# zgspose/PAVENet

Measured on AMD Instinct MI355X. Metric: clips/sec (T=7, 800x1344) fwd, higher is better.
Workload: dtype f32 (exact 3-term bf16 split on the bf16 MFMA)

## Files before the change

pavenet_amd/csrc/pave_gemm_dma.hip:

```cpp
#include <hip/hip_runtime.h>
#include <type_traits>
#include <stdint.h>

#include "pave_hip.h"
#include "pave_internal.h"
#include "pave_enc_math.h"

namespace {

typedef __bf16 bf16x8 __attribute__((ext_vector_type(8)));
typedef float f32x16 __attribute__((ext_vector_type(16)));
typedef unsigned u32x4 __attribute__((ext_vector_type(4)));
typedef float f32x4 __attribute__((ext_vector_type(4)));

constexpr int QBM = 128;
constexpr int QNS = 3;
constexpr int QCST = 36;

struct QConv {
  int H, W, Cin, Ho, Wo, stride;
  unsigned rcp;
};
struct QOut {
  float* out2;
// ... 125 lines not shown
}
#define PAVE_CLOCK_BEGIN(kind) diag_stagger(); const ClockStamp pave_cs(kind)
#define PAVE_CLOCK_END() pave_cs.end()
#define PAVE_PROBE_DROP_STORES() (g_diag_stagger == -1 || g_diag_stagger == -3 || g_diag_stagger == -5)
#define PAVE_PROBE_CACHED_A() (g_diag_stagger == -2 || g_diag_stagger == -3)
#define PAVE_PROBE_NO_CHAIN_SYNC() (g_diag_stagger == -4 || g_diag_stagger == -5)
#define PAVE_PROBE_NT_STORES() (g_diag_stagger == -6)
#define PAVE_PROBE_FREE_SPLIT() (g_diag_stagger == -7)
#else
#define PAVE_CLOCK_BEGIN(kind)
#define PAVE_CLOCK_END()
#define PAVE_PROBE_DROP_STORES() false
#define PAVE_PROBE_CACHED_A() false
#define PAVE_PROBE_NO_CHAIN_SYNC() false
#define PAVE_PROBE_NT_STORES() false
#define PAVE_PROBE_FREE_SPLIT() false
#endif

template <int TN, int WN, int KIND, bool ABIAS, bool LNORM, bool WIDE = false, int EPI = 0, int RM = 1, int PL = 3,
          bool HT = false, int IO = 0>
__device__ __forceinline__ void gemm_q_body(
    const float* __restrict__ A, const uint16_t* __restrict__ Wp, const float* __restrict__ bias,
    const float* residual, float* out, const int M, const int K, const int N, const int relu,
    const float* __restrict__ a_bias, const QConv g, const QOut os, const QLn ln,
    const float* __restrict__ A2 = nullptr, const int tile_m0 = -1, const int tile_n0 = 0,
    const QEpi* epi = nullptr) {
  constexpr int NWAVE = 4 * WN;
  constexpr int BN = WN * TN * 32;
  constexpr int BM = QBM * RM;
  constexpr bool AH = (IO & 1) != 0, OH = (IO & 2) != 0;
  static_assert(!AH || (PL == 1 && KIND == 0 && !ABIAS && RM == 1), "fp16 A rows: fp16 operand mode, plain rows");
  static_assert(!OH || (PL == 1 && !LNORM && EPI == 0 && !HT && RM == 1), "fp16 output: plain epilogue");
  constexpr int A_STAGE = AH ? BM * 32 : BM * 64;
  static_assert(RM == 1 || (RM == 2 && WN == 1 && !WIDE && !LNORM && EPI == 0), "two row tiles per wave: narrow form");
  static_assert(PL == 3 || PL == 1, "operand planes: 3 (bf16 split) or 1 (fp16)");
  constexpr int W_STAGE = PL * BN * 32;
  constexpr int STAGE = A_STAGE + W_STAGE;
  constexpr int NA = A_STAGE / 1024;
  constexpr int NWI = W_STAGE / 1024;
  constexpr int NDI = NA + NWI;
  constexpr int QMAX = (NDI + NWAVE - 1) / NWAVE;
  constexpr int QMIN = NDI / NWAVE;
  constexpr int QA = (NA + NWAVE - 1) / NWAVE;
  constexpr int NS = WIDE ? 2 : QNS;
  constexpr int EPI_OFF = 0;
  constexpr int STAT_OFF = NS * STAGE;
  constexpr int TQ = WIDE ? 2 : (HT ? 1 : TN);
  static_assert(!HT || (TN == 2 && WN == 1 && RM == 1 && !WIDE && !LNORM && EPI == 0 && PL == 3),
                "half-tail form: 64-column planes, one row tile per wave, 3 planes");
  static_assert(!WIDE || (TN == 8 && WN == 1 && !ABIAS), "wide form: 32 x 256 per wave");
  constexpr int ABOFF = STAT_OFF + (LNORM ? 2 * QBM * WN * 4 : 0);
  static_assert(NA % NWAVE == 0, "A DMA instructions divide evenly over the waves");
  static_assert(!LNORM || KIND == 0, "LayerNorm epilogue: plain row GEMM only");
  static_assert(KIND >= 0 && KIND <= 4, "row source");
  extern __shared__ __attribute__((aligned(1024))) unsigned char smem[];

  const int tid = threadIdx.x, lane = tid & 63;
  const int wave = __builtin_amdgcn_readfirstlane(tid >> 6);
  const int wm = wave / WN, wn = wave % WN;
  const int lr = lane & 31, kh = lane >> 5;
  const int ntiles = N / BN;
  const int ttot = ((M + BM - 1) / BM) * ntiles;
  const int per = ttot >> 3, rem = ttot & 7;
  const unsigned lds0 = (unsigned)(size_t)(__attribute__((address_space(3))) unsigned char*)smem;
  const int s0 = os.ks_slabs > 0 ? (int)blockIdx.y * os.ks_slabs : 0;
  const int nslabs = os.ks_slabs > 0 ? min(os.ks_slabs, K / 16 - s0) : K / 16;
  const long long w_slab = (long long)PL * N * 32;
  const unsigned char* const w_base = reinterpret_cast<const unsigned char*>(Wp);

  int m0 = 0, n0 = 0;
  unsigned a_voff[QA];
  unsigned a2_voff[QA];
  const unsigned char* a2_base = reinterpret_cast<const unsigned char*>(A2);
  int a_iy0[QA], a_ix0[QA];
  const float* a_img[QA];
  unsigned a_mask[QA];
  i32x4 a_rsrc;
  if (KIND == 1) {
    const unsigned long long ab = reinterpret_cast<unsigned long long>(A);
    a_rsrc.x = __builtin_amdgcn_readfirstlane((int)(unsigned)ab);
// ... 82 lines not shown
        dma16_buf(ok ? a_voff[q] + toff : 0xffffff00u, a_rsrc, dst);
      } else if (KIND == 2) {
        const int k0 = slab * 16;
        const int tap = k0 / g.Cin, c0 = k0 - tap * g.Cin;
        const int ky = tap / 3, kx = tap - ky * 3;
        const int iy = a_iy0[q] + ky, ix = a_ix0[q] + kx;
        const bool ok = tap < 9 && iy >= 0 && iy < g.H && ix >= 0 && ix < g.W;
        const float* src = ok ? a_img[q] + ((long long)iy * g.W + ix) * g.Cin + c0
                              : reinterpret_cast<const float*>(g_zero_chunk);
        dma16_flat(src, dst);
      } else if (KIND == 4) {
        const int s1 = g.Cin >> 4;
        if (slab < s1) dma16(a_voff[q], a_base + (long long)slab * 64, dst);
        else dma16(a2_voff[q], a2_base + (long long)(slab - s1) * 64, dst);
      } else {
        dma16(a_voff[q], a_base + (long long)slab * (AH ? 32 : 64), dst);
      }
    }
#pragma unroll
    for (int q = QA; q < QMAX; ++q) {
      const int j = wave + NWAVE * (q - QA);
      if (NWI % NWAVE == 0 || j < NWI)
        dma16(w_voff[q - QA], w_base + slab * w_slab, sl + A_STAGE + j * 1024);
    }
  };

  const int sw = (lr >> 2) & 3;
  const int a_rd0 = AH ? (wm * 32 + lr) * 32 + ((kh ^ ((lr >> 3) & 1)) * 16)
                       : (wm * 32 * RM + lr) * 64 + (((2 * kh) ^ sw) * 16);
  const int a_rd1 = a_rd0 ^ 16;
  const int w_rd = A_STAGE + (wn * TN * 32 + lr) * 32 + ((kh ^ ((lr >> 3) & 1)) * 16);

  f32x16 acc[RM * TN];
  f32x4 raw[RM][2];
  u32x4 apl[2][RM][PL];
  u32x4 wf[2][PL][TQ];
  const float* const ab_lds = reinterpret_cast<const float*>(smem + ABOFF);

  auto read_raw = [&](const int stage) {
    const unsigned char* st = smem + stage * STAGE;
#pragma unroll
    for (int rt = 0; rt < RM; ++rt) {
      raw[rt][0] = *reinterpret_cast<const f32x4*>(st + a_rd0 + rt * 2048);
      if constexpr (!AH) raw[rt][1] = *reinterpret_cast<const f32x4*>(st + a_rd1 + rt * 2048);
    }
  };
  auto read_wq = [&](const int stage, const int quarter, const int set) {
    const unsigned char* st = smem + stage * STAGE;
#pragma unroll
    for (int p = 0; p < PL; ++p)
#pragma unroll
      for (int j = 0; j < TQ; ++j)
        wf[set][p][j] =
            *reinterpret_cast<const u32x4*>(st + w_rd + (p * BN + (quarter * TQ + j) * 32) * 32);
  };
  u32x4 wtA[PL], wtB[PL], wt[PL];
  f32x4 acct[2];
  const int w_rdt = A_STAGE + (32 + (lane & 15)) * 32 + (((((lane >> 4) & 1)) ^ ((lane >> 3) & 1)) * 16);
  auto read_tail = [&](const int stage, u32x4 (&dst)[PL]) {
    const unsigned char* st = smem + stage * STAGE;
#pragma unroll
    for (int p = 0; p < PL; ++p) dst[p] = *reinterpret_cast<const u32x4*>(st + w_rdt + p * BN * 32);
  };
  auto read_frags = [&](const int stage, const int set) {
    read_raw(stage);
    read_wq(stage, 0, set);
    if constexpr (HT) {
      if (set == 0) read_tail(stage, wtA);
      else read_tail(stage, wtB);
    }
  };
  auto merge_tail = [&]() {
    if constexpr (HT) {
#pragma unroll
      for (int p = 0; p < PL; ++p)
#pragma unroll
        for (int i = 0; i < 4; ++i) wt[p][i] = lane < 32 ? wtA[p][i] : wtB[p][i];
    }
  };
  auto tail_pair = [&]() {
    if constexpr (HT) {
      typedef unsigned u32x2 __attribute__((ext_vector_type(2)));
#pragma unroll
      for (int p = 0; p < PL; ++p)
#pragma unroll
        for (int i = 0; i < 4; ++i) {
          u32x2 r = __builtin_amdgcn_permlane32_swap(apl[0][0][p][i], apl[1][0][p][i], false, false);
          r = __builtin_amdgcn_permlane16_swap(r.x, r.y, false, false);
          apl[0][0][p][i] = r.x, apl[1][0][p][i] = r.y;
        }
#pragma unroll
      for (int o = 2; o >= 0; --o)
#pragma unroll
        for (int pa = 0; pa <= o; ++pa)
#pragma unroll
          for (int hh = 0; hh < 2; ++hh)
            acct[hh] = __builtin_amdgcn_mfma_f32_16x16x32_bf16(
                __builtin_bit_cast(bf16x8, apl[hh][0][pa]), __builtin_bit_cast(bf16x8, wt[o - pa]), acct[hh], 0, 0, 0);
    }
  };
  auto split_raw = [&](const int slab, const int set) {
#pragma unroll
   for (int rt = 0; rt < RM; ++rt) {
    f32x4 lo = raw[rt][0], hi = raw[rt][1];
    if (ABIAS) {
      const f32x4 b0 = *reinterpret_cast<const f32x4*>(ab_lds + slab * 16 + kh * 8);
      const f32x4 b1 = *reinterpret_cast<const f32x4*>(ab_lds + slab * 16 + kh * 8 + 4);
#pragma unroll
      for (int i = 0; i < 4; ++i) {
        lo[i] = fmaxf(lo[i] + b0[i], 0.f);
        hi[i] = fmaxf(hi[i] + b1[i], 0.f);
      }
    }
    if constexpr (AH) {
      apl[set][rt][0] = __builtin_bit_cast(u32x4, lo);
    } else if constexpr (PL == 3) {
      if (PAVE_PROBE_FREE_SPLIT()) {
        apl[set][rt][0] = __builtin_bit_cast(u32x4, lo);
        apl[set][rt][1] = __builtin_bit_cast(u32x4, hi);
        apl[set][rt][2] = __builtin_bit_cast(u32x4, lo);
      } else
      split8(lo, hi, apl[set][rt]);
    } else {
      apl[set][rt][0] = u32x4{pack_rne_f16(lo.x, lo.y), pack_rne_f16(lo.z, lo.w), pack_rne_f16(hi.x, hi.y),
                              pack_rne_f16(hi.z, hi.w)};
    }
   }
  };
  auto mma = [&](const int set, const int o) {
    if constexpr (PL == 1) {
      if (o != 0) return;
#pragma unroll
      for (int rt = 0; rt < RM; ++rt)
#pragma unroll
        for (int j = 0; j < TQ; ++j)
          acc[rt * TN + j] = __builtin_amdgcn_mfma_f32_32x32x16_f16(
              __builtin_bit_cast(f16x8, apl[set][rt][0]), __builtin_bit_cast(f16x8, wf[set][0][j]),
              acc[rt * TN + j], 0, 0, 0);
    } else {
#pragma unroll
    for (int pa = 0; pa <= o; ++pa)
#pragma unroll
      for (int rt = 0; rt < RM; ++rt)
#pragma unroll
        for (int j = 0; j < TQ; ++j) {
          acc[rt * TN + j] = __builtin_amdgcn_mfma_f32_32x32x16_bf16(
              __builtin_bit_cast(bf16x8, apl[set][rt][pa]), __builtin_bit_cast(bf16x8, wf[set][o - pa][j]),
              acc[rt * TN + j], 0, 0, 0);
        }
    }
  };
  auto mma_q = [&](const int aset, const int wset, const int quarter) {
    if constexpr (PL == 1) {
#pragma unroll
      for (int j = 0; j < TQ; ++j)
        acc[quarter * TQ + j] = __builtin_amdgcn_mfma_f32_32x32x16_f16(
            __builtin_bit_cast(f16x8, apl[aset][0][0]), __builtin_bit_cast(f16x8, wf[wset][0][j]),
            acc[quarter * TQ + j], 0, 0, 0);
    } else
#pragma unroll
    for (int o = 2; o >= 0; --o)
#pragma unroll
      for (int pa = 0; pa <= o; ++pa)
#pragma unroll
        for (int j = 0; j < TQ; ++j) {
          acc[quarter * TQ + j] = __builtin_amdgcn_mfma_f32_32x32x16_bf16(
              __builtin_bit_cast(bf16x8, apl[aset][0][pa]),
              __builtin_bit_cast(bf16x8, wf[wset][o - pa][j]), acc[quarter * TQ + j], 0, 0, 0);
        }
  };

  constexpr int NPS = 4;
  const int erow = lane >> 3, ec4 = lane & 7;
  constexpr int NPR = NPS * RM;
  constexpr int NT = RM * TN;
  constexpr int RB = WIDE ? 4 : TN;
  float4 resv[RB][NPS];
  constexpr unsigned kOut = 0x80000000u;
  using u32x4 = unsigned int __attribute__((ext_vector_type(4)));
  unsigned rro[NPR];
  __amdgpu_buffer_rsrc_t rrs;
  auto residual_rows = [&](const int em0) {
    const bool table = os.res_rows != 0;
    const int rows_left = min(BM, M - em0);
    rrs = __builtin_amdgcn_make_buffer_rsrc(
        const_cast<float*>(residual) + (table ? 0ll : (long long)em0 * os.n_real), 0,
        (table ? os.res_rows : rows_left) * os.n_real * 4, 0x00020000);
    const int lrow0 = wm * 32 * RM + erow;
    const bool stepwise = os.res_rows >= 32 * RM;
    const unsigned rbase = table ? (unsigned)(em0 + lrow0) % (unsigned)os.res_rows : 0u;
#pragma unroll
    for (int ps = 0; ps < NPR; ++ps) {
      unsigned rr = (unsigned)(lrow0 + ps * 8);
      if (table) {
        if (stepwise) {
          rr = rbase + ps * 8;
          if (rr >= (unsigned)os.res_rows) rr -= (unsigned)os.res_rows;
        } else {
          rr = (unsigned)(em0 + lrow0 + ps * 8) % (unsigned)os.res_rows;
        }
      }
      rro[ps] = lrow0 + ps * 8 < rows_left ? rr * (unsigned)(os.n_real * 4) + ec4 * 16 : kOut;
    }
  };
  auto prefetch_residual_tile = [&](const int en0, const int t, const int buf) {
    const int rt = t / TN, j = t % TN;
    const int ncol0 = en0 + wn * TN * 32 + j * 32;
    const bool colok = WIDE || ncol0 + ec4 * 4 < os.n_real;
#pragma unroll
    for (int ps = 0; ps < NPS; ++ps)
      resv[buf][ps] = __builtin_bit_cast(
          float4, __builtin_amdgcn_raw_buffer_load_b128(rrs, colok ? rro[rt * NPS + ps] : kOut, ncol0 * 4, 0));
  };
  auto prefetch_residual = [&](const int em0, const int en0) {
    if (!residual) return;
    residual_rows(em0);
#pragma unroll
    for (int j = 0; j < RB; ++j) prefetch_residual_tile(en0, j, j);
  };

  if (ABIAS) {
    float* ab = reinterpret_cast<float*>(smem + ABOFF);
    for (int i = tid; i < K; i += 64 * NWAVE) ab[i] = a_bias[i];
  }
  setup_tile(blockIdx.x);
  {
    const int em0 = m0, en0 = n0;
    if constexpr (!WIDE) {
      issue(0, 0);
      issue(1, 1);
      issue(2, 2);
#pragma unroll
      for (int j = 0; j < NT; ++j)
#pragma unroll
        for (int r = 0; r < 16; ++r) acc[j][r] = 0.f;
      acct[0] = f32x4{0.f, 0.f, 0.f, 0.f}, acct[1] = acct[0];
      PAVE_QWAIT(2 * QMIN);
      read_frags(0, 0);
      split_raw(0, 0);

#define PAVE_QSTEP(I, FULL)                                                    \
  if (FULL || s + I < nslabs - 1) {                                            \
    constexpr int cur = (I) & 1, nxt = cur ^ 1;                                \
    const int sl = s + I;                                                      \
    if (FULL || sl + 2 < nslabs) PAVE_QWAIT(QMIN); else PAVE_QWAIT(0);         \
    if (FULL || sl + 3 < nslabs) issue(sl + 3, (I) % 3);                       \
    read_frags(((I) + 1) % 3, nxt);                                            \
    __builtin_amdgcn_sched_barrier(0);                                         \
    mma(cur, 2);                                                               \
    if (HT && cur == 0) merge_tail();                                          \
    if (!(HT && cur == 1)) split_raw(sl + 1, nxt);                             \
    mma(cur, 1);                                                               \
    mma(cur, 0);                                                               \
    if (HT && cur == 1) {    \
      tail_pair();                                                             \
      split_raw(sl + 1, nxt);                                                  \
    }                                                                          \
  }
      int s = 0;
      for (; s + 9 <= nslabs; s += 6) {
        PAVE_QSTEP(0, true)
// ... 414 lines not shown
};
__device__ __forceinline__ void chain_sync() {
  if (PAVE_PROBE_NO_CHAIN_SYNC()) return;
  __builtin_amdgcn_fence(__ATOMIC_RELEASE, "workgroup");
  __builtin_amdgcn_s_barrier();
  __builtin_amdgcn_fence(__ATOMIC_ACQUIRE, "workgroup");
}
template <bool HAS_A, int KIND2, int CN, int RMC = 1, int PL = 3>
__global__ __launch_bounds__(256) __attribute__((amdgpu_waves_per_eu(2, 2))) void bottleneck_chain_kernel(
    const ChainArgs p) {
  const QLn ln0{nullptr, nullptr, 0.f};
  constexpr int CBM = QBM * RMC;
  const int ttot = (p.M + CBM - 1) / CBM;
  const int per = ttot >> 3, rem = ttot & 7;
  const int xcd = blockIdx.x & 7, idx = blockIdx.x >> 3;
  const int tm0 = (xcd * per + (xcd < rem ? xcd : rem) + idx) * CBM;
  PAVE_CLOCK_BEGIN(4);
  if constexpr (HAS_A) {
    gemm_q_body<2, 1, 1, false, false, false, 0, RMC, PL>(p.c1, p.w2, p.b2, nullptr, p.c2, p.M, 576, 64, 1, nullptr,
                                                      QConv{p.H, p.W, 64, p.H, p.W, 1, 1u << 30},
                                                      QOut{nullptr, 0, 0, 64, 0}, ln0, nullptr, tm0, 0);
    chain_sync();
  }
#pragma unroll
  for (int h = 0; h < RMC; ++h) {
    if (h > 0) PAVE_QBAR();
    if (tm0 + h * QBM < p.M)
      gemm_q_body<8, 1, KIND2, false, false, true, 0, 1, PL>(p.c2, p.w3, p.b3, p.residual, p.out, p.M, p.K3, 256, 1,
                                                   nullptr, QConv{0, 0, p.k1, 0, 0, 0},
                                                   QOut{nullptr, 0, 0, 256, 0}, ln0, p.a2, tm0 + h * QBM, 0);
  }
  if constexpr (CN > 0) {
    chain_sync();
    if constexpr (CN == 64 && RMC == 2) {
      gemm_q_body<2, 1, 0, false, false, false, 0, 2, PL>(
          p.out, p.w1n, p.b1n, nullptr, p.c1n, p.M, 256, CN, 1, nullptr, QConv{0, 0, 0, 0, 0, 0},
          QOut{nullptr, 0, 0, CN, 0}, ln0, nullptr, tm0, 0);
    } else {
#pragma unroll
      for (int h = 0; h < RMC; ++h) {
        if (h > 0) PAVE_QBAR();
        if (tm0 + h * QBM < p.M)
          gemm_q_body<(CN > 0 ? CN / 32 : 2), 1, 0, false, false, false, 0, 1, PL>(
              p.out, p.w1n, p.b1n, nullptr, p.c1n, p.M, 256, CN, 1, nullptr, QConv{0, 0, 0, 0, 0, 0},
              QOut{nullptr, 0, 0, CN, 0}, ln0, nullptr, tm0 + h * QBM, 0);
      }
    }
  }
  PAVE_CLOCK_END();
}

template <int PL>
__global__ __launch_bounds__(512) __attribute__((amdgpu_waves_per_eu(2, 2))) void gemm_q_ln_kernel(
    const float* __restrict__ A, const uint16_t* __restrict__ Wp, const float* __restrict__ bias,
    const float* residual, float* out, const int M, const int K, const int N, const QLn ln) {
  PAVE_CLOCK_BEGIN(5);
  gemm_q_body<4, 2, 0, false, true, false, 0, 1, PL>(A, Wp, bias, residual, out, M, K, N, 0, nullptr,
                                                     QConv{0, 0, 0, 0, 0, 0}, QOut{nullptr, 0, 0, N, 0}, ln);
  PAVE_CLOCK_END();
}

template <int PL, int IO = 0>
__global__ __launch_bounds__(256) __attribute__((amdgpu_waves_per_eu(2, 2))) void gemm_w_ln_kernel(
    const float* __restrict__ A, const uint16_t* __restrict__ Wp, const float* __restrict__ bias,
    const float* residual, float* out, const int M, const int K, const int N, const QLn ln) {
  PAVE_CLOCK_BEGIN(6);
  gemm_q_body<8, 1, 0, false, true, true, 0, 1, PL, false, IO>(A, Wp, bias, residual, out, M, K, N, 0, nullptr,
                                                               QConv{0, 0, 0, 0, 0, 0}, QOut{nullptr, 0, 0, N, 0}, ln);
  PAVE_CLOCK_END();
}
// ... 115 lines not shown
      const int col = j * 32 + ec4 * 4;
      const float4 b4 = bias ? *reinterpret_cast<const float4*>(bias + col) : make_float4(0.f, 0.f, 0.f, 0.f);
#pragma unroll
      for (int i = 0; i < 16; ++i) Cs[((i & 3) + 8 * (i >> 2) + 4 * kh) * QCST + lr] = acc[r][j][i];
      __builtin_amdgcn_fence(__ATOMIC_RELEASE, "wavefront");
      __builtin_amdgcn_wave_barrier();
      __builtin_amdgcn_fence(__ATOMIC_ACQUIRE, "wavefront");
#pragma unroll
      for (int ps = 0; ps < 4; ++ps) {
        const int lrow = ps * 8 + erow;
        const int ox = ox0 + wave * 32 + lrow;
        float4 v = *reinterpret_cast<const float4*>(Cs + lrow * QCST + ec4 * 4);
        v.x += b4.x, v.y += b4.y, v.z += b4.z, v.w += b4.w;
        if (relu) {
          v.x = fmaxf(v.x, 0.f), v.y = fmaxf(v.y, 0.f), v.z = fmaxf(v.z, 0.f), v.w = fmaxf(v.w, 0.f);
        }
        if (ox < Wo && oy + r < Ho) *reinterpret_cast<float4*>(orow + (long long)ox * 64 + col) = v;
      }
      __builtin_amdgcn_fence(__ATOMIC_RELEASE, "wavefront");
      __builtin_amdgcn_wave_barrier();
    }
  }
  PAVE_CLOCK_END();
}

template <int TN, int KIND, bool ABIAS, int RM = 1, int PL = 3, bool HT = false>
int launch_q(const float* a, const uint16_t* w, const float* bias, const float* residual, float* out,
             long long M, int K, int N, int relu, const float* a_bias, hipStream_t st, const QConv g,
             const QOut os, const float* a2 = nullptr, int ksplit = 1) {
  constexpr int BN = TN * 32;
  constexpr int BM = QBM * RM;
  constexpr int STAGE = BM * 64 + PL * BN * 32;
  constexpr int EPIB = 4 * 32 * QCST * 4;
  const int smem = (QNS * STAGE > EPIB ? QNS * STAGE : EPIB) + (ABIAS ? K * 4 : 0);
  const long long gx = ((M + BM - 1) / BM) * (N / BN);
  if (gx >= (1ll << 31)) return pave_internal_fail(PAVE_E_ARG, "gemm_q: grid too large");
  return pave_launch_lds<gemm_q_kernel<TN, KIND, ABIAS, RM, PL, HT>>(
      "gemm_q: cannot raise dynamic LDS limit", dim3((unsigned)gx, (unsigned)ksplit), dim3(256), smem, st, a, w, bias,
      residual, out, (int)M, K, N, relu, a_bias, g, os, a2);
}

__global__ __launch_bounds__(256) void splitk_reduce_kernel(
    const float* __restrict__ ws, const int parts, const long long total4, const int n4,
    const float* __restrict__ bias, const float* __restrict__ residual, const int relu,
    float* __restrict__ out) {
  const long long i = (long long)blockIdx.x * 256 + threadIdx.x;
  if (i >= total4) return;
  const float4* w4 = reinterpret_cast<const float4*>(ws);
  float4 v = w4[i];
  for (int p = 1; p < parts; ++p) {
    const float4 t = w4[p * total4 + i];
    v.x += t.x, v.y += t.y, v.z += t.z, v.w += t.w;
  }
  if (bias) {
    const float4 b = reinterpret_cast<const float4*>(bias)[i % n4];
    v.x += b.x, v.y += b.y, v.z += b.z, v.w += b.w;
  }
  if (residual) {
    const float4 r = reinterpret_cast<const float4*>(residual)[i];
    v.x += r.x, v.y += r.y, v.z += r.z, v.w += r.w;
  }
  if (relu) v.x = fmaxf(v.x, 0.f), v.y = fmaxf(v.y, 0.f), v.z = fmaxf(v.z, 0.f), v.w = fmaxf(v.w, 0.f);
  reinterpret_cast<float4*>(out)[i] = v;
}

template <int TN, int PF, int PL = 3>
__global__ __launch_bounds__(256) void gemm_s_kernel(
// ... 502 lines not shown
                                  dv == PAVE_DV_CONV3_ADDR64);
#define PAVE_QGO(TN_)                                                                               \
  if (kind == 0) {                                                                                  \
    if (a_bias) return launch_q<TN_, 0, true, 1, PL>(a, w, bias, residual, out, M, K, N, relu, a_bias, st, g, os); \
    return launch_q<TN_, 0, false, 1, PL>(a, w, bias, residual, out, M, K, N, relu, a_bias, st, g, os, nullptr, ksplit); \
  }                                                                                                 \
  if (kind == 1 && big3) return launch_q<TN_, 2, false, 1, PL>(a, w, bias, residual, out, M, K, N, relu, a_bias, st, g, os, nullptr, ksplit); \
  if (kind == 1) return launch_q<TN_, 1, false, 1, PL>(a, w, bias, residual, out, M, K, N, relu, a_bias, st, g, os, nullptr, ksplit); \
  if (kind == 4) return launch_q<TN_, 4, false, 1, PL>(a, w, bias, residual, out, M, K, N, relu, a_bias, st, g, os, a2, ksplit); \
  return launch_q<TN_, 3, false, 1, PL>(a, w, bias, residual, out, M, K, N, relu, a_bias, st, g, os, nullptr, ksplit)
  const long long wtiles = ((M + QBM - 1) / QBM) * (N / 256) * ksplit;
  if (N % 256 == 0 && n_real == N && !narrow && !a_bias && dv != PAVE_DV_WIDE_NEVER &&
      (wtiles >= 400 || dv == PAVE_DV_WIDE_ALWAYS) &&
      !(kind == 0 && W > 0 && W % 256 != 0) && (!out2 || n_split % 256 == 0)) {
    if (kind == 0) return launch_w<0, PL>(a, w, bias, residual, out, M, K, N, relu, st, g, os, nullptr, ksplit);
    if (kind == 1 && big3) return launch_w<2, PL>(a, w, bias, residual, out, M, K, N, relu, st, g, os, nullptr, ksplit);
    if (kind == 1) return launch_w<1, PL>(a, w, bias, residual, out, M, K, N, relu, st, g, os, nullptr, ksplit);
    if (kind == 4) return launch_w<4, PL>(a, w, bias, residual, out, M, K, N, relu, st, g, os, a2, ksplit);
    return launch_w<3, PL>(a, w, bias, residual, out, M, K, N, relu, st, g, os, nullptr, ksplit);
  }
  if (kind == 0 && N % 256 == 128 && N >= 384 && n_real == N && !narrow && !a_bias && dv != PAVE_DV_WIDE_NEVER &&
      W == 0 && ksplit == 1 && (((M + QBM - 1) / QBM) * (N / 256 + 1) >= 400 || dv == PAVE_DV_WIDE_ALWAYS) &&
      (!out2 || n_split % 256 == 0))
    return launch_wn<PL>(a, w, bias, residual, out, M, K, N, relu, st, g, os);
  if (N == 128 && n_real <= 96 && n_real > 64 && !narrow && !out2 && dv != PAVE_DV_WIDE_NEVER &&
      ksplit == 1 && (kind == 1 || kind == 0) && !a_bias) {
    if (kind == 1 && big3) return launch_q<3, 2, false, 1, PL>(a, w, bias, residual, out, M, K, N, relu, a_bias, st, g, os);
    if (kind == 1 && dv != PAVE_DV_RM2_NEVER && (((M + 255) / 256) >= 1024 || dv == PAVE_DV_RM2_ALWAYS) &&
        (os.res_rows == 0 || os.res_rows >= 64))
      return launch_q<3, 1, false, 2, PL>(a, w, bias, residual, out, M, K, N, relu, a_bias, st, g, os);
    if (kind == 1) return launch_q<3, 1, false, 1, PL>(a, w, bias, residual, out, M, K, N, relu, a_bias, st, g, os);
    return launch_q<3, 0, false, 1, PL>(a, w, bias, residual, out, M, K, N, relu, a_bias, st, g, os);
  }
  if (N % 128 == 0 && !narrow) { PAVE_QGO(4); }
  if (N % 64 == 0 && (kind == 0 || (kind == 1 && !big3)) && !a_bias && ksplit == 1 && dv == PAVE_DV_RM2_ALWAYS &&
      (os.res_rows == 0 || os.res_rows >= 64) && (long long)N * 1024 < (1ll << 31)) {
    if (kind == 1) return launch_q<2, 1, false, 2, PL>(a, w, bias, residual, out, M, K, N, relu, a_bias, st, g, os);
    return launch_q<2, 0, false, 2, PL>(a, w, bias, residual, out, M, K, N, relu, a_bias, st, g, os);
  }
  if constexpr (PL == 3) {
    if (N == 64 && n_real > 32 && n_real <= 48 && kind == 1 && !big3 && !a_bias && !out2 && ksplit == 1 &&
        dv != PAVE_DV_NO_HALF_TAIL && dv != PAVE_DV_RM2_NEVER &&
        dv != PAVE_DV_RM2_ALWAYS)
      return launch_q<2, 1, false, 1, 3, true>(a, w, bias, residual, out, M, K, N, relu, a_bias, st, g, os);
  }
  if (N % 64 == 0) { PAVE_QGO(2); }
#undef PAVE_QGO
  return pave_internal_fail(PAVE_E_ARG, "gemm_q: N %% 64 == 0 required");
}

int pave_internal_gemm_q(const GemmQ& q) {
  return pave_with_planes(q.planes, "gemm_q: 3 bf16 planes or 1 fp16 plane",
                          [&](auto pl) { return gemm_q_dispatch<decltype(pl)::value>(q); });
}

template <int PL>
static int gemm_encproj_go(const float* a, const void* w_planes, const float* table, long long table_rows,
                           const float* value_bias, const float* ref, const int* levels_hw, float* value,
                           float* samp, long long M, int K, void* stream) {
  if (K % 32 != 0 || K < 64 || K >= (1 << 23)) return pave_internal_fail(PAVE_E_ARG, "gemm_encproj: K %% 32 == 0, 64 <= K < 2^23");
  QEpi epi{};
  epi.ref = ref;
  for (int l = 0; l < 4; ++l) {
    if (levels_hw[2 * l] <= 0 || levels_hw[2 * l + 1] <= 0)
      return pave_internal_fail(PAVE_E_ARG, "gemm_encproj: bad level size");
    epi.fH[l] = (float)levels_hw[2 * l], epi.fW[l] = (float)levels_hw[2 * l + 1];
// ... 79 lines not shown
  const long long gx = ((M + QBM - 1) / QBM) * (N / 256);
  if (gx >= (1ll << 31)) return pave_internal_fail(PAVE_E_ARG, "gemm_fp16_act: grid too large");
  const dim3 grid((unsigned)gx), block(256);
  constexpr const char* what = "gemm_fp16_act: cannot raise dynamic LDS limit";
  if (gamma) {
    const QLn ln{gamma, beta, eps};
    if (a_f16)
      return pave_launch_lds<gemm_w_ln_kernel<1, 1>>(what, grid, block, w_smem<1>(), st, af, w, bias, residual, of,
                                                     (int)M, K, N, ln);
    return pave_launch_lds<gemm_w_ln_kernel<1, 0>>(what, grid, block, w_smem<1>(), st, af, w, bias, residual, of,
                                                   (int)M, K, N, ln);
  }
  const QConv g0{};
  const QOut os{nullptr, 0, 0, N, 0};
  const float* const none = nullptr;
  switch ((a_f16 ? 1 : 0) | (out_f16 ? 2 : 0)) {
    case 0:
      return pave_launch_lds<gemm_w_kernel<0, 1, 0>>(what, grid, block, w_smem<1>(), st, af, w, bias, none, of, (int)M,
                                                     K, N, relu, g0, os, none);
    case 1:
      return pave_launch_lds<gemm_w_kernel<0, 1, 1>>(what, grid, block, w_smem<1>(), st, af, w, bias, none, of, (int)M,
                                                     K, N, relu, g0, os, none);
    case 2:
      return pave_launch_lds<gemm_w_kernel<0, 1, 2>>(what, grid, block, w_smem<1>(), st, af, w, bias, none, of, (int)M,
                                                     K, N, relu, g0, os, none);
    default:
      return pave_launch_lds<gemm_w_kernel<0, 1, 3>>(what, grid, block, w_smem<1>(), st, af, w, bias, none, of, (int)M,
                                                     K, N, relu, g0, os, none);
  }
}

template <bool HAS_A, int KIND2, int CN, int RMC = 1, int PL = 3>
static int launch_chain(const ChainArgs& p, hipStream_t st) {
  constexpr int smem = RMC == 2 ? (3 * (2 * QBM * 64 + 3 * 64 * 32) > W_SMEM ? 3 * (2 * QBM * 64 + 3 * 64 * 32) : W_SMEM) : W_SMEM;
  constexpr int CBM = QBM * RMC;
  return pave_launch_lds<bottleneck_chain_kernel<HAS_A, KIND2, CN, RMC, PL>>(
      "bottleneck_chain: cannot raise dynamic LDS limit", dim3((unsigned)((p.M + CBM - 1) / CBM)), dim3(256), smem, st, p);
}

template <int PL>
static int bottleneck_chain_go(const float* c1, const void* w2_planes, const float* b2, float* c2,
                               const void* w3_planes, const float* b3, const float* residual,
                               const float* a2, int k2, float* out, const void* w1n_planes,
                               const float* b1n, float* c1n, int cn, int N, int H, int W,
                               void* stream) {
  if (!c2 || !w3_planes || !out || (c1 != nullptr) != (w2_planes != nullptr))
    return pave_internal_fail(PAVE_E_ARG, "bottleneck_chain: null pointer (c1 and w2_planes: both or neither)");
  if (N <= 0 || H <= 0 || W <= 0 || (long long)N * H * W >= (1ll << 31) ||
      (c1 && (long long)N * H * W * 64 * 4 >= (1ll << 32) - 65536))
    return pave_internal_fail(PAVE_E_ARG, "bottleneck_chain: bad sizes (N*H*W < 2^31; with the 3x3 inside "
                                          "the launch the c1 map must stay below 4 GiB)");
  if ((a2 != nullptr) != (k2 > 0) || (a2 && (k2 % 32 != 0 || k2 > 960)) || (a2 && residual))
    return pave_internal_fail(PAVE_E_ARG, "bottleneck_chain: a2 [M, k2] (k2 %% 32 == 0) replaces the residual");
  if ((w1n_planes != nullptr) != (cn > 0) || (w1n_planes && (!c1n || (cn != 64 && cn != 128))))
    return pave_internal_fail(PAVE_E_ARG, "bottleneck_chain: next conv1 with 64 or 128 output channels, or none");
  const int dvc = pave_internal_diag_variant();
  if (dvc == PAVE_DV_FIRST_GEN)
    return pave_internal_fail(PAVE_E_UNSUPPORTED, "bottleneck_chain: LDS-DMA generation only");
  ChainArgs p{c1, static_cast<const uint16_t*>(w2_planes), b2, c2,
              static_cast<const uint16_t*>(w3_planes), b3, residual, a2, out,
              static_cast<const uint16_t*>(w1n_planes), b1n, c1n,
              N * H * W, H, W, 64 + k2, 64};
  hipStream_t st = reinterpret_cast<hipStream_t>(stream);
#define PAVE_CHAIN_GO(HA)                                              \
  if (a2) {                                                            \
    if (cn == 64) return launch_chain<HA, 4, 64, 1, PL>(p, st);               \
    if (cn == 128) return launch_chain<HA, 4, 128, 1, PL>(p, st);             \
    return launch_chain<HA, 4, 0, 1, PL>(p, st);                              \
  }                                                                    \
  if (cn == 64) return launch_chain<HA, 0, 64, 1, PL>(p, st);                 \
  if (cn == 128) return launch_chain<HA, 0, 128, 1, PL>(p, st);               \
  return launch_chain<HA, 0, 0, 1, PL>(p, st)
  if (c1 && cn > 0 && dvc != PAVE_DV_RM2_NEVER && (p.M >= 256 * 1024 || dvc == PAVE_DV_RM2_ALWAYS)) {
    if (a2) {
      if (cn == 64) return launch_chain<true, 4, 64, 2, PL>(p, st);
      return launch_chain<true, 4, 128, 2, PL>(p, st);
    }
    if (cn == 64) return launch_chain<true, 0, 64, 2, PL>(p, st);
    return launch_chain<true, 0, 128, 2, PL>(p, st);
  }
  if (c1) { PAVE_CHAIN_GO(true); }
  PAVE_CHAIN_GO(false);
#undef PAVE_CHAIN_GO
}

#ifdef PAVE_DIAG
extern "C" int pave_diag_clock_reset(void) {
  unsigned long long z[16] = {};
  return hipMemcpyToSymbol(HIP_SYMBOL(g_clock_acc), z, sizeof(z)) == hipSuccess ? PAVE_OK : PAVE_E_LAUNCH;
}
extern "C" int pave_diag_set_stagger(int v) {
  if (hipDeviceSynchronize() != hipSuccess) return PAVE_E_LAUNCH;
  return hipMemcpyToSymbol(HIP_SYMBOL(g_diag_stagger), &v, sizeof(v)) == hipSuccess ? PAVE_OK : PAVE_E_LAUNCH;
}
extern "C" int pave_diag_hwid_read(unsigned* out1024) {
  if (!out1024) return PAVE_E_ARG;
  if (hipDeviceSynchronize() != hipSuccess) return PAVE_E_LAUNCH;
  return hipMemcpyFromSymbol(out1024, HIP_SYMBOL(g_diag_hwid), 1024 * sizeof(unsigned)) == hipSuccess
             ? PAVE_OK : PAVE_E_LAUNCH;
}
extern "C" int pave_diag_clock_read(unsigned long long* out16) {
  if (!out16) return PAVE_E_ARG;
  if (hipDeviceSynchronize() != hipSuccess) return PAVE_E_LAUNCH;
  return hipMemcpyFromSymbol(out16, HIP_SYMBOL(g_clock_acc), 16 * sizeof(unsigned long long)) == hipSuccess
             ? PAVE_OK : PAVE_E_LAUNCH;
// ... 33 lines not shown
```

pavenet_amd/csrc/pave_internal.h:

```cpp
#ifndef PAVE_INTERNAL_H_
#define PAVE_INTERNAL_H_
#include <type_traits>

int pave_internal_fail(int code, const char* msg);

template <auto KERN, class... A>
inline int pave_launch(dim3 grid, dim3 block, int smem, hipStream_t st, A... args) {
  hipLaunchKernelGGL(KERN, grid, block, smem, st, args...);
  const hipError_t e = hipGetLastError();
  if (e != hipSuccess) return pave_internal_fail(PAVE_E_LAUNCH, hipGetErrorString(e));
  return PAVE_OK;
}
template <auto KERN, class... A>
inline int pave_launch_lds(const char* refusal, dim3 grid, dim3 block, int smem, hipStream_t st, A... args) {
  static int raised = 0;
  if (smem > raised) {
    if (hipFuncSetAttribute(reinterpret_cast<const void*>(KERN), hipFuncAttributeMaxDynamicSharedMemorySize,
                            smem) != hipSuccess)
      return pave_internal_fail(PAVE_E_LAUNCH, refusal);
    raised = smem;
  }
  return pave_launch<KERN>(grid, block, smem, st, args...);
}

enum PaveDiag : int {
  PAVE_DV_NONE = 0,
  PAVE_DV_TILE256 = 2,
  PAVE_DV_W8_ALWAYS = 3,
  PAVE_DV_W8_NEVER = 4,
  PAVE_DV_CONV3_ADDR64 = 5,
  PAVE_DV_NO_SPLITK = 6,
  PAVE_DV_WIDE_ALWAYS = 7,
  PAVE_DV_WIDE_NEVER = 8,
  PAVE_DV_FIRST_GEN = 9,
  PAVE_DV_LN_8WAVE = 13,
  PAVE_DV_LN_WIDE = 14,
  PAVE_DV_RM2_NEVER = 15,
  PAVE_DV_RM2_ALWAYS = 16,
  PAVE_DV_NO_HALF_TAIL = 17,
  PAVE_DV_SWIN_PER_LANE = 18,
  PAVE_DV_SMALL_ROWS_R5 = 19,
  PAVE_DV_WIDE_ONE_PER_CU = 20,
  PAVE_DV_SK_ANY_ROWS = 21,
};
#ifdef PAVE_DIAG
int pave_internal_diag_variant();
#else
static inline int pave_internal_diag_variant() { return PAVE_DV_NONE; }
#endif

static inline int q_planes(int nplanes) { return nplanes == 3 ? 3 : (nplanes == PAVE_PLANES_FP16 ? 1 : 0); }
template <class F>
inline int pave_with_planes(int planes, const char* refusal, F f) {
  if (planes == 1) return f(std::integral_constant<int, 1>{});
  if (planes != 3) return pave_internal_fail(PAVE_E_ARG, refusal);
  return f(std::integral_constant<int, 3>{});
}

enum GemmQRows : int {
  GEMMQ_ROWS = 0,
  GEMMQ_CONV3X3 = 1,
  GEMMQ_CONV1X1S = 3,
  GEMMQ_ROWS2 = 4,
};
struct GemmQ {
  GemmQRows rows = GEMMQ_ROWS;
  const float* a = nullptr;
  const float* a2 = nullptr;
  const float* a_bias = nullptr;
  const void* w_planes = nullptr;
  const float* bias = nullptr;
  const float* residual = nullptr;
  long long residual_rows = 0;
  float* out = nullptr;
  float* out2 = nullptr;
  int n_split = 0;
// ... 30 lines not shown
```

Measured before the change: 59.24.

## Add tall GEMM tile forms with 4x2 or 2x4 accumulator tiles per wave

Adds a 'tall' form of the bf16-split GEMM in which each wave holds 4x2 or 2x4 32x32 accumulator tiles (BM up to 512 rows), with double-buffered stages and a new software-pipelined slab loop that interleaves per-row-tile A reads, splits and MFMAs. The goal is to reuse weight fragments across more row tiles and so cut the LDS traffic per MFMA. By default it is chosen only for N==128 plain or 3x3 rows with many row tiles; the other forms and the bottleneck-chain use sit behind a diagnostic switch. In exchange it uses more accumulator registers, which risks lower occupancy, and has only two pipeline stages.

```diff
diff --git a/pavenet_amd/csrc/pave_gemm_dma.hip b/pavenet_amd/csrc/pave_gemm_dma.hip
--- a/pavenet_amd/csrc/pave_gemm_dma.hip
+++ b/pavenet_amd/csrc/pave_gemm_dma.hip
@@ -181,7 +181,13 @@
   static_assert(!AH || (PL == 1 && KIND == 0 && !ABIAS && RM == 1), "fp16 A rows: fp16 operand mode, plain rows");
   static_assert(!OH || (PL == 1 && !LNORM && EPI == 0 && !HT && RM == 1), "fp16 output: plain epilogue");
   constexpr int A_STAGE = AH ? BM * 32 : BM * 64;
-  static_assert(RM == 1 || (RM == 2 && WN == 1 && !WIDE && !LNORM && EPI == 0), "two row tiles per wave: narrow form");
+  constexpr bool TALL = !WIDE && RM > 1 && RM * TN == 8;
+  static_assert(RM == 1 || TALL || (RM == 2 && WN == 1 && !WIDE && !LNORM && EPI == 0),
+                "two row tiles per wave: narrow form");
+  static_assert(!TALL || (((RM == 4 && TN == 2) || (RM == 2 && TN == 4)) && WN == 1 && PL == 3 && (KIND == 0 || KIND == 1) &&
+                          !ABIAS && !LNORM && EPI == 0 && !HT && IO == 0),
+                "tall forms: 4 x 2 or 2 x 4 accumulator tiles per wave, 3 planes, plain rows or the buffer-addressed "
+                "3x3, plain epilogue (bias / residual / ReLU), no a_bias / LayerNorm / EPI / half tail / fp16 IO");
   static_assert(PL == 3 || PL == 1, "operand planes: 3 (bf16 split) or 1 (fp16)");
   constexpr int W_STAGE = PL * BN * 32;
   constexpr int STAGE = A_STAGE + W_STAGE;
@@ -191,10 +197,11 @@
   constexpr int QMAX = (NDI + NWAVE - 1) / NWAVE;
   constexpr int QMIN = NDI / NWAVE;
   constexpr int QA = (NA + NWAVE - 1) / NWAVE;
-  constexpr int NS = WIDE ? 2 : QNS;
+  constexpr int NS = (WIDE || TALL) ? 2 : QNS;
   constexpr int EPI_OFF = 0;
   constexpr int STAT_OFF = NS * STAGE;
-  constexpr int TQ = WIDE ? 2 : (HT ? 1 : TN);
+  constexpr int TQ = (WIDE || TALL) ? 2 : (HT ? 1 : TN);
+  constexpr int RMH = TALL ? 1 : RM;
   static_assert(!HT || (TN == 2 && WN == 1 && RM == 1 && !WIDE && !LNORM && EPI == 0 && PL == 3),
                 "half-tail form: 64-column planes, one row tile per wave, 3 planes");
   static_assert(!WIDE || (TN == 8 && WN == 1 && !ABIAS), "wide form: 32 x 256 per wave");
@@ -343,18 +350,23 @@
   const int w_rd = A_STAGE + (wn * TN * 32 + lr) * 32 + ((kh ^ ((lr >> 3) & 1)) * 16);
 
   f32x16 acc[RM * TN];
-  f32x4 raw[RM][2];
-  u32x4 apl[2][RM][PL];
+  f32x4 raw[RMH][2];
+  u32x4 apl[2][RMH][PL];
   u32x4 wf[2][PL][TQ];
   const float* const ab_lds = reinterpret_cast<const float*>(smem + ABOFF);
 
   auto read_raw = [&](const int stage) {
     const unsigned char* st = smem + stage * STAGE;
 #pragma unroll
-    for (int rt = 0; rt < RM; ++rt) {
+    for (int rt = 0; rt < RMH; ++rt) {
       raw[rt][0] = *reinterpret_cast<const f32x4*>(st + a_rd0 + rt * 2048);
       if constexpr (!AH) raw[rt][1] = *reinterpret_cast<const f32x4*>(st + a_rd1 + rt * 2048);
     }
+  };
+  auto read_raw_rt = [&](const int stage, const int rt) {
+    const unsigned char* st = smem + stage * STAGE;
+    raw[0][0] = *reinterpret_cast<const f32x4*>(st + a_rd0 + rt * 2048);
+    raw[0][1] = *reinterpret_cast<const f32x4*>(st + a_rd1 + rt * 2048);
   };
   auto read_wq = [&](const int stage, const int quarter, const int set) {
     const unsigned char* st = smem + stage * STAGE;
@@ -412,7 +424,7 @@
   };
   auto split_raw = [&](const int slab, const int set) {
 #pragma unroll
-   for (int rt = 0; rt < RM; ++rt) {
+   for (int rt = 0; rt < RMH; ++rt) {
     f32x4 lo = raw[rt][0], hi = raw[rt][1];
     if (ABIAS) {
       const f32x4 b0 = *reinterpret_cast<const f32x4*>(ab_lds + slab * 16 + kh * 8);
@@ -478,6 +490,18 @@
           acc[quarter * TQ + j] = __builtin_amdgcn_mfma_f32_32x32x16_bf16(
               __builtin_bit_cast(bf16x8, apl[aset][0][pa]),
               __builtin_bit_cast(bf16x8, wf[wset][o - pa][j]), acc[quarter * TQ + j], 0, 0, 0);
+        }
+  };
+  auto mma_t = [&](const int aset, const int wset, const int rt, const int half) {
+#pragma unroll
+    for (int o = 2; o >= 0; --o)
+#pragma unroll
+      for (int pa = 0; pa <= o; ++pa)
+#pragma unroll
+        for (int j = 0; j < TQ; ++j) {
+          acc[rt * TN + half * TQ + j] = __builtin_amdgcn_mfma_f32_32x32x16_bf16(
+              __builtin_bit_cast(bf16x8, apl[aset][0][pa]), __builtin_bit_cast(bf16x8, wf[wset][o - pa][j]),
+              acc[rt * TN + half * TQ + j], 0, 0, 0);
         }
   };
 
@@ -537,7 +561,64 @@
   setup_tile(blockIdx.x);
   {
     const int em0 = m0, en0 = n0;
-    if constexpr (!WIDE) {
+    if constexpr (TALL) {
+      issue(0, 0);
+      issue(1, 1);
+#pragma unroll
+      for (int j = 0; j < NT; ++j)
+#pragma unroll
+        for (int r = 0; r < 16; ++r) acc[j][r] = 0.f;
+      PAVE_QWAIT(QMIN);
+      read_wq(0, 0, 0);
+      read_raw_rt(0, 0);
+      split_raw(0, 0);
+      if constexpr (RM == 2) read_raw_rt(0, 1);
+#define PAVE_T012(cur)                                                         \
+  if constexpr (RM == 4) {                                                     \
+    read_raw_rt(cur, 1);                                                       \
+    mma_t(0, cur, 0, 0);                                                       \
+    split_raw(0, 1);                                                           \
+    read_raw_rt(cur, 2);                                                       \
+    mma_t(1, cur, 1, 0);                                                       \
+    split_raw(0, 0);                                                           \
+    read_raw_rt(cur, 3);                                                       \
+    mma_t(0, cur, 2, 0);                                                       \
+    split_raw(0, 1);                                                           \
+  } else {                                                                     \
+    read_wq(cur, 1, 1);                                                        \
+    mma_t(0, 0, 0, 0);                                                         \
+    split_raw(0, 1);                                                           \
+    mma_t(1, 0, 1, 0);                                                         \
+    mma_t(0, 1, 0, 1);                                                         \
+  }                                                                            \
+  PAVE_QWAIT(0);
+#define PAVE_T3(cur, nxt)                                                      \
+  read_wq(nxt, 0, RM == 4 ? nxt : 0);                                          \
+  read_raw_rt(nxt, 0);                                                         \
+  __builtin_amdgcn_sched_barrier(0);                                           \
+  mma_t(1, RM == 4 ? cur : 1, RM - 1, RM == 4 ? 0 : 1);                        \
+  split_raw(0, 0);                                                             \
+  if constexpr (RM == 2) read_raw_rt(nxt, 1);
+#define PAVE_TSTEP(I)                                                          \
+  {                                                                            \
+    constexpr int cur = (I) & 1, nxt = cur ^ 1;                                \
+    PAVE_T012(cur)                                                             \
+    issue(s + I + 2, cur);                                                     \
+    PAVE_T3(cur, nxt)                                                          \
+  }
+      for (int s = 0; s + 4 <= nslabs; s += 2) {
+        PAVE_TSTEP(0)
+        PAVE_TSTEP(1)
+      }
+      PAVE_T012(0)
+      PAVE_T3(0, 1)
+      PAVE_T012(1)
+      prefetch_residual(em0, en0);
+      mma_t(1, 1, RM - 1, RM == 4 ? 0 : 1);
+#undef PAVE_T012
+#undef PAVE_T3
+#undef PAVE_TSTEP
+    } else if constexpr (!WIDE) {
       issue(0, 0);
       issue(1, 1);
       issue(2, 2);
@@ -1018,10 +1099,19 @@
   }
   if constexpr (CN > 0) {
     chain_sync();
-    if constexpr (CN == 64 && RMC == 2) {
-      gemm_q_body<2, 1, 0, false, false, false, 0, 2, PL>(
+    if constexpr (CN == 64 && RMC >= 2) {
+      gemm_q_body<2, 1, 0, false, false, false, 0, RMC, PL>(
           p.out, p.w1n, p.b1n, nullptr, p.c1n, p.M, 256, CN, 1, nullptr, QConv{0, 0, 0, 0, 0, 0},
           QOut{nullptr, 0, 0, CN, 0}, ln0, nullptr, tm0, 0);
+    } else if constexpr (CN == 128 && RMC == 4) {
+#pragma unroll
+      for (int h = 0; h < 2; ++h) {
+        if (h > 0) PAVE_QBAR();
+        if (tm0 + h * 2 * QBM < p.M)
+          gemm_q_body<4, 1, 0, false, false, false, 0, 2, PL>(
+              p.out, p.w1n, p.b1n, nullptr, p.c1n, p.M, 256, CN, 1, nullptr, QConv{0, 0, 0, 0, 0, 0},
+              QOut{nullptr, 0, 0, CN, 0}, ln0, nullptr, tm0 + h * 2 * QBM, 0);
+      }
     } else {
 #pragma unroll
       for (int h = 0; h < RMC; ++h) {
@@ -1203,7 +1293,8 @@
   constexpr int BM = QBM * RM;
   constexpr int STAGE = BM * 64 + PL * BN * 32;
   constexpr int EPIB = 4 * 32 * QCST * 4;
-  const int smem = (QNS * STAGE > EPIB ? QNS * STAGE : EPIB) + (ABIAS ? K * 4 : 0);
+  constexpr int NS = (RM > 1 && RM * TN == 8) ? 2 : QNS;
+  const int smem = (NS * STAGE > EPIB ? NS * STAGE : EPIB) + (ABIAS ? K * 4 : 0);
   const long long gx = ((M + BM - 1) / BM) * (N / BN);
   if (gx >= (1ll << 31)) return pave_internal_fail(PAVE_E_ARG, "gemm_q: grid too large");
   return pave_launch_lds<gemm_q_kernel<TN, KIND, ABIAS, RM, PL, HT>>(
@@ -1772,6 +1863,20 @@
     if (kind == 1) return launch_q<3, 1, false, 1, PL>(a, w, bias, residual, out, M, K, N, relu, a_bias, st, g, os);
     return launch_q<3, 0, false, 1, PL>(a, w, bias, residual, out, M, K, N, relu, a_bias, st, g, os);
   }
+  if constexpr (PL == 3) {
+    const bool tall_ok = (kind == 0 || (kind == 1 && !big3)) && (kind != 0 || (H > 0 ? H : K) < (1 << 21)) && !a_bias && !out2 &&
+                         ksplit == 1 && n_real == N && (os.res_rows == 0 || os.res_rows >= 128) &&
+                         (long long)N * 2048 < (1ll << 31) && dv != PAVE_DV_TALL_NEVER;
+    if (tall_ok && N % 128 == 0 && !narrow &&
+        (dv == PAVE_DV_TALL_ALWAYS || (N == 128 && W <= 0 && (M + 255) / 256 >= 1024))) {
+      if (kind == 1) return launch_q<4, 1, false, 2, 3>(a, w, bias, residual, out, M, K, N, relu, a_bias, st, g, os);
+      return launch_q<4, 0, false, 2, 3>(a, w, bias, residual, out, M, K, N, relu, a_bias, st, g, os);
+    }
+    if (tall_ok && N % 64 == 0 && (N % 128 != 0 || narrow) && dv == PAVE_DV_TALL_ALWAYS) {
+      if (kind == 1) return launch_q<2, 1, false, 4, 3>(a, w, bias, residual, out, M, K, N, relu, a_bias, st, g, os);
+      return launch_q<2, 0, false, 4, 3>(a, w, bias, residual, out, M, K, N, relu, a_bias, st, g, os);
+    }
+  }
   if (N % 128 == 0 && !narrow) { PAVE_QGO(4); }
   if (N % 64 == 0 && (kind == 0 || (kind == 1 && !big3)) && !a_bias && ksplit == 1 && dv == PAVE_DV_RM2_ALWAYS &&
       (os.res_rows == 0 || os.res_rows >= 64) && (long long)N * 1024 < (1ll << 31)) {
@@ -1917,7 +2022,8 @@
 
 template <bool HAS_A, int KIND2, int CN, int RMC = 1, int PL = 3>
 static int launch_chain(const ChainArgs& p, hipStream_t st) {
-  constexpr int smem = RMC == 2 ? (3 * (2 * QBM * 64 + 3 * 64 * 32) > W_SMEM ? 3 * (2 * QBM * 64 + 3 * 64 * 32) : W_SMEM) : W_SMEM;
+  constexpr int smem64 = RMC == 4 ? 2 * (4 * QBM * 64 + PL * 64 * 32) : (RMC == 2 ? 3 * (2 * QBM * 64 + 3 * 64 * 32) : 0);
+  constexpr int smem = smem64 > W_SMEM ? smem64 : W_SMEM;
   constexpr int CBM = QBM * RMC;
   return pave_launch_lds<bottleneck_chain_kernel<HAS_A, KIND2, CN, RMC, PL>>(
       "bottleneck_chain: cannot raise dynamic LDS limit", dim3((unsigned)((p.M + CBM - 1) / CBM)), dim3(256), smem, st, p);
@@ -1956,6 +2062,16 @@
   if (cn == 64) return launch_chain<HA, 0, 64, 1, PL>(p, st);                 \
   if (cn == 128) return launch_chain<HA, 0, 128, 1, PL>(p, st);               \
   return launch_chain<HA, 0, 0, 1, PL>(p, st)
+  if constexpr (PL == 3) {
+    if (c1 && cn > 0 && dvc == PAVE_DV_TALL_ALWAYS) {
+      if (a2) {
+        if (cn == 64) return launch_chain<true, 4, 64, 4, 3>(p, st);
+        return launch_chain<true, 4, 128, 4, 3>(p, st);
+      }
+      if (cn == 64) return launch_chain<true, 0, 64, 4, 3>(p, st);
+      return launch_chain<true, 0, 128, 4, 3>(p, st);
+    }
+  }
   if (c1 && cn > 0 && dvc != PAVE_DV_RM2_NEVER && (p.M >= 256 * 1024 || dvc == PAVE_DV_RM2_ALWAYS)) {
     if (a2) {
       if (cn == 64) return launch_chain<true, 4, 64, 2, PL>(p, st);
diff --git a/pavenet_amd/csrc/pave_internal.h b/pavenet_amd/csrc/pave_internal.h
--- a/pavenet_amd/csrc/pave_internal.h
+++ b/pavenet_amd/csrc/pave_internal.h
@@ -42,6 +42,8 @@
   PAVE_DV_SMALL_ROWS_R5 = 19,
   PAVE_DV_WIDE_ONE_PER_CU = 20,
   PAVE_DV_SK_ANY_ROWS = 21,
+  PAVE_DV_TALL_NEVER = 22,
+  PAVE_DV_TALL_ALWAYS = 23,
 };
 #ifdef PAVE_DIAG
 int pave_internal_diag_variant();
```

New measurement: 59.33, median of 6. No clear change (+0.2%).
